# proycon/analiticcl

Hardware: AMD Instinct MI355X
Metric: scored (query,candidate) pairs/sec + queries/sec, 200k-lexicon, len≤16, 1/2/4/8 GPU (higher is better)
Workload: dtype u8

## Files before the change

analiticcl_amd/csrc/engine.hip:

```cpp
#include <hip/hip_runtime.h>

#include <algorithm>
#include <atomic>
#include <functional>
#include <chrono>
#include <cmath>
#include <cstdio>
#include <cstdlib>
#include <cstring>
#include <map>
#include <memory>
#include <mutex>
#include <unordered_map>
#include <numeric>
#include <thread>
#include <type_traits>

#include "engine_internal.h"

namespace anx {

#define HIP_TRY(expr)                                                                          \
  do {                                                                                         \
    hipError_t _e = (expr);                                                                    \
// ... 372 lines not shown
  DeviceLexicon* d = new DeviceLexicon();
  d->device = device;
  { DevPool& pl = pool_of(device); std::lock_guard<std::mutex> g(pl.mu); ++pl.lexicons; }
  d->nplanes = img.nplanes;
  d->nsym = img.nsym;
  d->nclasses = img.nclasses;
  d->nentries = img.nentries;
  d->cstride = img.cstride;
  d->any_variants = img.any_variants ? 1 : 0;
  uint32_t maxlen = 1;
  for (uint32_t m : img.ent_meta) maxlen = std::max(maxlen, m & 0xFFu);
  d->max_len = maxlen;
  int rc = ANX_OK;
  std::vector<EntRec> rec(img.ent_vocab.size());
  for (size_t e = 0; e < rec.size(); ++e) rec[e] = EntRec{img.ent_vocab[e], img.ent_freq[e], img.ent_order[e], img.ent_meta[e]};
  std::vector<uint4> erec(2 * img.ent_vocab.size());
  for (size_t e = 0; e < img.ent_vocab.size(); ++e) {
    memcpy(&erec[2 * e], &img.rows[(size_t)img.ent_rowoff[e] * 16], 16);
    erec[2 * e + 1] = make_uint4(img.ent_meta[e], img.ent_rowoff[e], img.ent_freq[e], 0u);
  }
  std::vector<uint4> eplanes(img.ent_vocab.size());
  for (size_t e = 0; e < img.ent_vocab.size(); ++e) {
    uint32_t pw[3];
    symbol_planes16(&img.rows[(size_t)img.ent_rowoff[e] * 16], img.ent_meta[e] & 0xFFu, pw);
    eplanes[e] = make_uint4(img.ent_meta[e], pw[0], pw[1], pw[2]);
  }
  std::vector<uint4> srec((size_t)img.nentries + 1, make_uint4(0u, 0u, 0u, 0u));
  std::vector<uint2> srec34((size_t)img.nentries + 1, make_uint2(0u, 0u));
  for (uint32_t c = 0; c < img.nclasses; ++c)
    for (uint32_t e = img.cls_off[c]; e < img.cls_off[c + 1]; ++e) {
      srec[e] = make_uint4(img.cls_bits[c], img.cls_bits[(size_t)img.cstride + c], img.cls_len[c], c);
      srec34[e] = make_uint2(img.cls_bits[2 * (size_t)img.cstride + c], img.cls_bits[3 * (size_t)img.cstride + c]);
    }
  srec[img.nentries] = make_uint4(0u, 0u, 255u, 0xFFFFFFFFu);
// ... 922 lines not shown
    if (surv_fill) {
      CompactArgs ca{m.have_freq ? 1 : 0, dl->any_variants};
      hipLaunchKernelGGL(k_compact, dim3(((surv_fill + 255) / 256) * SCAN_REGIONS), dim3(256), 0, st, b->surv, b->sctr,
                         (uint32_t)b->surv_region_cap, ca, b->qcur, dl->ent_rec, dl->ent_var_off, dl->var_target,
                         dl->var_target_freq, dl->var_score, b->c_rows);
    }
  } else if (b->surv_cap == 0 && (rc = ensure_surv(b, b->hint_rows ? b->hint_rows : (size_t)nq * 16 / cap_div() + 1024, err))) return rc;
  const uint32_t row_cap = (uint32_t)std::min<size_t>(b->surv_cap, 0xFFFFFFFFu);
  if (!dl->any_variants)
    hipLaunchKernelGGL(k_compact_grouped, dim3(COMPACT_P * SCAN_REGIONS), dim3(COMPACT_B), 0, st, b->surv, b->sctr,
                       (uint32_t)b->surv_region_cap, m.have_freq ? 1 : 0, b->qcur, dl->ent_rec, b->c_rows, b->soff + nq, row_cap,
                       b->counters + CTR_OVERFLOW);
  HIP_TRY(hipEventRecord(b->ev[3], st));
  if (b->conf_mode == 2 && (rc = conf_launch(m, dl, b, st, true, row_cap, err))) return rc;
  launch_rank(ra, st, nq, b->soff, b->c_rows, b->qmaxfreq, b->qexpand, b->t_key, b->r_rows, b->r_count, dl->any_variants ? 0xFFFFFFFFu : row_cap, b->counters + CTR_OVERFLOW,
              dl->any_variants ? SegRows{nullptr, 0u, nullptr} : SegRows{so.seg, so.seg_cap, dl->ent_rec});
  if (b->conf_mode == 1 && (rc = conf_launch(m, dl, b, st, false, row_cap, err))) return rc;
  exclusive_scan(b->r_count, nq, b->r_off, b->scan_tmp, st, b->counters + CTR_MAXROWS);
  HIP_TRY(hipEventRecord(b->ev[4], st));
  return ANX_OK;
}

int Run::readback() {
  HIP_TRY(hipMemcpyAsync(b->h_read + HR_SCTR, b->sctr, SCAN_REGIONS * RC_STRIDE * sizeof(uint32_t), hipMemcpyDeviceToHost, st));
  HIP_TRY(hipMemcpyAsync(b->h_read + HR_LCTR, b->lctr, 3 * SCAN_REGIONS * RC_STRIDE * sizeof(uint32_t), hipMemcpyDeviceToHost, st));
  HIP_TRY(hipMemcpyAsync(b->h_read + HR_CTR, b->counters, CTR_N * sizeof(uint32_t), hipMemcpyDeviceToHost, st));
  HIP_TRY(hipMemcpyAsync(b->h_read + HR_TOTAL_SURV, b->soff + nq, sizeof(uint32_t), hipMemcpyDeviceToHost, st));
  HIP_TRY(hipMemcpyAsync(b->h_read + HR_TOTAL_RESULTS, b->r_off + nq, sizeof(uint32_t), hipMemcpyDeviceToHost, st));
  b->h_read[HR_CONF] = b->h_read[HR_CONF + 1] = 0;
  if (b->conf_mode && b->cf_ctr) HIP_TRY(hipMemcpyAsync(b->h_read + HR_CONF, b->cf_ctr, 2 * sizeof(uint32_t), hipMemcpyDeviceToHost, st));
  HIP_TRY(hipEventRecord(b->ev_done, st));
// ... 476 lines not shown
```

analiticcl_amd/csrc/host_model.cpp:

```cpp
#include "host_model.h"
#include "adjacency.h"

#include <sched.h>

#include <thread>

#include <algorithm>
#include <cmath>
#include <cstdio>
#include <cstring>
#include <fstream>
#include <numeric>
#include <sstream>

#include "unicode_tables.inc"

namespace anx {

static std::vector<uint32_t> make_primes() {
  std::vector<uint32_t> p;
  for (uint32_t n = 2; p.size() < 168; ++n) {
    bool prime = true;
    for (uint32_t d : p) {
      if (d * d > n) break;
// ... 488 lines not shown

namespace {
struct SwitchDef { const char* name; void (*set)(Switches&, const char*); };
int flag01(const char* v, int dflt) { return !v ? dflt : (v[0] == '0' ? 0 : 1); }
const SwitchDef kSwitches[] = {
    {"ANX_ENCODE", [](Switches& s, const char* v) { s.encode_host = v && strcmp(v, "host") == 0; }},
    {"ANX_SCAN", [](Switches& s, const char* v) { s.scan_sad = v && strcmp(v, "sad") == 0; }},
    {"ANX_SCAN_WALK", [](Switches& s, const char* v) { s.scan_walk_flat = v && strcmp(v, "flat") == 0; }},
    {"ANX_SCAN_TQ", [](Switches& s, const char* v) { const int x = v ? atoi(v) : 0; s.scan_tq = x >= 1 && x <= 64 ? x : 0; }},
    {"ANX_SCAN_ADJ", [](Switches& s, const char* v) { s.scan_adj = flag01(v, 1); }},
    {"ANX_ADJ_BUILD", [](Switches& s, const char* v) { s.adj_build_host = v && strcmp(v, "host") == 0; }},
    {"ANX_ADJ_CLOSURE", [](Switches& s, const char* v) { const int x = v ? atoi(v) : 2; s.adj_closure = x >= 0 && x <= kAdjMaxClosure ? x : kAdjMaxClosure; }},
    {"ANX_SCAN_CHUNK_FUSED", [](Switches& s, const char* v) { const int x = v ? atoi(v) : 0; s.scan_chunk_fused = x >= 32 && x <= 1024 ? x : 0; }},
    {"ANX_ADJ_FAIL", [](Switches& s, const char* v) { s.adj_fail = flag01(v, 0); }},
    {"ANX_SMALL", [](Switches& s, const char* v) { s.small_path = flag01(v, 1); }},
    {"ANX_SURV_SEG", [](Switches& s, const char* v) { const int x = v ? atoi(v) : 32; s.surv_seg = x >= 0 && x <= 256 ? x : 32; }},
    {"ANX_ENC_PRIORITY", [](Switches& s, const char* v) { s.enc_priority = flag01(v, 1); }},
    {"ANX_HINTS", [](Switches& s, const char* v) { s.hints = flag01(v, 1); }},
    {"ANX_ADJ_MB", [](Switches& s, const char* v) { const long x = v ? atol(v) : 0; s.adj_budget_mb = x > 0 ? x : 16384; }},
    {"ANX_SIG_GROUPS", [](Switches& s, const char* v) { const int x = v ? atoi(v) : 0; s.sig_groups = x >= 1 && x <= 8 ? x : 0; }},
    {"ANX_PREFILTER", [](Switches& s, const char* v) { s.prefilter = flag01(v, 1); }},
    {"ANX_SCORE_FAST", [](Switches& s, const char* v) { s.score_fast = flag01(v, 1); }},
    {"ANX_FS_SPLIT", [](Switches& s, const char* v) { s.fs_split = flag01(v, 1); }},
    {"ANX_FS_PLANES", [](Switches& s, const char* v) { s.fs_planes = flag01(v, 1); }},
    {"ANX_FS_B7", [](Switches& s, const char* v) { s.fs_b7 = flag01(v, 1); }},
    {"ANX_SCAN_FUSE", [](Switches& s, const char* v) { s.fuse_prefilter = flag01(v, 1); }},
    {"ANX_CAP_DIV", [](Switches& s, const char* v) { const long x = v ? atol(v) : 0; s.cap_div = x > 1 ? x : 1; }},
    {"ANX_MAX_BATCH", [](Switches& s, const char* v) { const long x = v ? atol(v) : 0; s.max_batch = x > 0 ? x : (4l << 20); }},
    {"ANX_RUN_OVERLAP", [](Switches& s, const char* v) { s.run_overlap = (v && atoi(v) == 0 && v[0] == '0') ? 0 : 1; }},
    {"ANX_SHARD_POLICY", [](Switches& s, const char* v) { s.shard_by_length = (v && strcmp(v, "range") == 0) ? 0 : 1; }},
// ... 184 lines not shown
    std::vector<uint32_t> byval(lex.nclasses);
    std::iota(byval.begin(), byval.end(), 0u);
    std::sort(byval.begin(), byval.end(), [&](uint32_t a, uint32_t b) { return lex.cls_value[a].cmp(lex.cls_value[b]) < 0; });
    lex.ent_order.assign(lex.nentries, 0);
    uint32_t pos = 0;
    for (uint32_t r : byval)
      for (uint32_t e = lex.cls_off[r]; e < lex.cls_off[r + 1]; ++e) lex.ent_order[e] = pos++;
  }
  for (int c = 0; c <= kMaxSymbols; ++c) lex.bucket_begin[c + 1] += lex.bucket_begin[c];
  for (int c = 0; c <= kMaxSymbols; ++c) lex.siglen_begin[c + 1] += lex.siglen_begin[c];
  lex.nsigs = (uint32_t)lex.sig_lo.size();
  const size_t nsig_pad = ((size_t)lex.nsigs + 63) / 64 * 64 + 64;
  lex.sig_lo.resize(nsig_pad, 0xFFFFFFFFu);
  lex.sig_hi.resize(nsig_pad, 0xFFFFFFFFu);
  lex.sig_cbeg.resize(nsig_pad + 1, lex.nclasses);
  build_lm();
  index_generation.fetch_add(1, std::memory_order_release);
  built = true;
  return ANX_OK;
}

bool HostModel::into_ngram(uint64_t vocab_id, std::vector<uint64_t>& out) const {
  out.clear();
  if (vocab_id >= decoder.size()) return false;
  const std::string& text = decoder[vocab_id].text;
  const size_t tokencount = (size_t)std::count(text.begin(), text.end(), ' ') + 1;
  if (tokencount > 5) return false;
  size_t pos = 0;
  for (;;) {
    const size_t e = text.find(' ', pos);
    const std::string tok = text.substr(pos, e == std::string::npos ? std::string::npos : e - pos);
    auto it = encoder.find(tok);
    out.push_back(it == encoder.end() ? 2 : it->second);
    if (e == std::string::npos) break;
// ... 74 lines not shown
```

analiticcl_amd/csrc/host_model.h:

```cpp
#pragma once
#include <cstdint>
#include <atomic>
#include <memory>
#include <mutex>
#include <string>
#include <unordered_map>
#include <vector>

#include "../../include/anx.h"
#include "confusables_core.hpp"
#include "contextrules_flat.hpp"

namespace anx {

constexpr int kMaxSymbols = 255;
constexpr int kMaxAlphabet = 166;
constexpr int kMaxAnagramDistance = 12;
constexpr int kMaxEditDistance = 12;

struct AlphabetMember {
  std::string bytes;
  int nchars;
};

// ... 50 lines not shown
  int search_onepass = 1;
  int scan_chunk_fused = 0;
  int adj_fail = 0;
  int small_path = 1;
  int enc_priority = 1;
  int hints = 1;
  int encode_timing = 0;
  int search_timing = 0;
  int search_parts = 4;
  long search_parts_min = 2l << 20;
  long search_part_bytes = 4l << 20;
  int search_prio = 1;
  int search_early_output = 1;
  int search_first_pct = 50;
  int surv_seg = 32;
  int learn_fold_host = 0;
  int learn_hash_bits = 63;
};
Switches& switches();
bool set_switch(const char* name, const char* value);

struct VariantRef {
  bool variant_of;
  uint64_t id;
  double score;
};

struct VocabEntry {
  std::string text;
  std::vector<uint8_t> norm;
// ... 13 lines not shown
  std::string to_decimal() const;
};

struct LexiconImage {
  int nsym = 0;
  int nplanes = 0;
  uint32_t nclasses = 0, nentries = 0;
  std::vector<uint32_t> cls_planes;
  uint32_t cstride = 0;
  std::vector<uint32_t> cls_bits;
  std::vector<uint8_t> cls_len;
  std::vector<uint32_t> cls_off;
  uint32_t bucket_begin[kMaxSymbols + 2];
  std::vector<uint32_t> ent_vocab;
  std::vector<uint32_t> ent_freq;
  std::vector<uint32_t> ent_meta;
  std::vector<uint32_t> ent_var_off;
  std::vector<uint32_t> var_target;
  std::vector<uint32_t> var_target_freq;
  std::vector<double> var_score;
  bool any_variants = false;
  std::vector<uint32_t> ent_rowoff;
  std::vector<uint32_t> ent_order;
  std::vector<uint8_t> rows;
  std::vector<BigVal> cls_value;
  std::vector<uint8_t> sym_group;
  uint32_t nsigs = 0;
  std::vector<uint32_t> sig_lo, sig_hi;
  std::vector<uint32_t> sig_cbeg;
  uint32_t siglen_begin[kMaxSymbols + 2];
// ... 129 lines not shown
```

analiticcl_amd/csrc/index_cache.cpp:

```cpp
#include <algorithm>
#include <cstdio>
#include <cstring>

#include "host_model.h"

namespace anx {
namespace {

constexpr char kMagic[8] = {'A', 'N', 'X', 'I', 'D', 'X', '0', '3'};

struct Writer {
  FILE* f;
  bool ok = true;
  void raw(const void* p, size_t n) { if (ok && n && fwrite(p, 1, n, f) != n) ok = false; }
  template <typename T> void pod(const T& v) { raw(&v, sizeof v); }
  void str(const std::string& s) { pod<uint64_t>(s.size()); raw(s.data(), s.size()); }
  template <typename T> void vec(const std::vector<T>& v) { pod<uint64_t>(v.size()); raw(v.data(), v.size() * sizeof(T)); }
};
struct Reader {
  FILE* f;
  bool ok = true;
  void raw(void* p, size_t n) { if (ok && n && fread(p, 1, n, f) != n) ok = false; }
  template <typename T> void pod(T& v) { raw(&v, sizeof v); }
  void str(std::string& s) {
// ... 157 lines not shown
    lex = LexiconImage();
    built = false;
    err = path + " is truncated or corrupt";
    return ANX_EIO;
  }
  encoder.clear();
  encoder.reserve(decoder.size() * 2);
  for (size_t id = 0; id < decoder.size(); ++id) encoder.emplace(decoder[id].text, (uint64_t)id);
  class_of_cv.clear();
  class_of_cv.reserve((size_t)x.nclasses * 2);
  std::string cv((size_t)x.nplanes * 4, '\0');
  for (uint32_t c = 0; c < x.nclasses; ++c) {
    for (int p = 0; p < x.nplanes; ++p) memcpy(&cv[(size_t)p * 4], &x.cls_planes[(size_t)p * x.cstride + c], 4);
    class_of_cv.emplace(cv, c);
  }
  build_lm();
  index_generation.fetch_add(1, std::memory_order_release);
  built = true;
  return ANX_OK;
}

int index_read_tag(const std::string& path, std::string* tag, std::string& err) {
  FILE* f = fopen(path.c_str(), "rb");
  if (!f) { err = "cannot open " + path; return ANX_EIO; }
  Reader r{f};
  char magic[8];
  r.raw(magic, sizeof magic);
  uint32_t groups = 0;
  r.pod(groups);
  std::string fp;
// ... 9 lines not shown
```

analiticcl_amd/csrc/kernels_common.hpp:

```cpp
#pragma once

struct Tile {
  uint32_t q0, nq;
  uint32_t s0, s1;
  uint32_t k;
  uint32_t lq;
  uint32_t sig_lo, sig_hi;
  uint32_t kind;
  uint32_t d;
  uint32_t kend;
  uint32_t ball0, balln;
  uint32_t adj;
  uint32_t flags;
};
constexpr uint32_t BALL_MAX = 4096;
constexpr uint32_t SIG_BYTE_MAX = 120;

constexpr int kSymbolPlanesMaxA = 61;
__host__ __device__ inline void symbol_planes16(const uint8_t* row, uint32_t len, uint32_t (&w)[3]) {
  uint32_t p[6] = {0u, 0u, 0u, 0u, 0u, 0u};
  for (uint32_t i = 0; i < 16u && i < len; ++i) {
    const uint32_t v = (uint32_t)row[i] + 1u;
    for (uint32_t b = 0; b < 6u; ++b) p[b] |= ((v >> b) & 1u) << i;
  }
// ... 73 lines not shown
  uint4* sig = nullptr;
  uint32_t* sig_cbeg = nullptr;
  uint32_t* ent_vocab = nullptr;
  uint32_t* ent_freq = nullptr;
  uint32_t* ent_meta = nullptr;
  uint32_t* ent_rowoff = nullptr;
  uint32_t* ent_order = nullptr;
  EntRec* ent_rec = nullptr;
  uint4* e_rec = nullptr;
  uint4* e_planes = nullptr;
  uint32_t* ent_var_off = nullptr;
  uint32_t* var_target = nullptr;
  uint32_t* var_target_freq = nullptr;
  double* var_score = nullptr;
  int any_variants = 0;
  uint4* rows = nullptr;
  DevAlphabet alpha;
  size_t bytes = 0;
  double* quot = nullptr;
  mutable RunHints hints;
  mutable struct DeviceLm* dlm = nullptr;
  mutable struct DeviceConf* dconf = nullptr;
};

enum { CTR_SKIPPED = 2, CTR_MAXROWS = 3 , CTR_OVERFLOW = 4 , CTR_N = 8 };

struct SurvRow {
  double score;
  unsigned long long ord;
  uint32_t vocab, freq;
  uint32_t via, pad;
};
struct SurvRec {
  uint32_t q, e;
  double score;
};
struct SurvSeg {
  double score;
  uint32_t e, pad;
};
struct DevRow {
  uint32_t vocab_id, via;
  double dist_score, freq_score;
};

struct Batch {
  int device = 0;
  size_t nq = 0;
  anx_params params;
  std::vector<uint32_t> order;
  std::vector<int32_t> status;
  size_t n_input = 0;
  std::vector<Tile> tiles;
  uint32_t ntiles = 0;
  uint32_t n_sad_tiles = 0;
// ... 97 lines not shown
```

analiticcl_amd/csrc/kernels_rank.hpp:

```cpp
#pragma once

struct CompactArgs {
  int have_freq, any_variants;
};
__global__ __launch_bounds__(256) void k_compact(const SurvRec* __restrict__ surv, const uint32_t* __restrict__ sctr,
                                                 uint32_t region_cap, CompactArgs a,
                                                 uint32_t* __restrict__ qcur, const EntRec* __restrict__ ent_rec,
                                                 const uint32_t* __restrict__ ent_var_off,
                                                 const uint32_t* __restrict__ var_target,
                                                 const uint32_t* __restrict__ var_target_freq,
                                                 const double* __restrict__ var_score, SurvRow* __restrict__ c_rows) {
  const uint32_t region = blockIdx.x % SCAN_REGIONS, i = (blockIdx.x / SCAN_REGIONS) * 256 + threadIdx.x;
  const bool live = i < sctr[region * RC_STRIDE];
  if (!live) return;
  const SurvRec sr = surv[(size_t)region * region_cap + i];
  const double s = sr.score;
  const uint32_t e = sr.e, q = sr.q;
  const EntRec er = ent_rec[e];
  const uint32_t f = a.have_freq ? er.freq : 1u;
  const unsigned long long ord = (unsigned long long)er.order << 20;
  uint32_t v0 = 0, v1 = 0, self = 1;
  if (a.any_variants) {
    v0 = ent_var_off[e];
    v1 = ent_var_off[e + 1];
// ... 104 lines not shown
  }
}

struct RankArgs {
  double cutoff_threshold;
  uint64_t max_matches;
  float freq_weight;
  int have_freq, any_variants;
};
constexpr int RANK_LCAP = 128;

struct SegRows {
  const SurvSeg* seg;
  uint32_t cap;
  const EntRec* ent_rec;
};
__device__ __forceinline__ SurvRow row_of(const SurvRow* __restrict__ c_rows, const SegRows& sr, int have_freq, uint32_t q, uint32_t seg0, uint32_t i) {
  if (i < sr.cap) {
    const uint4 g = *reinterpret_cast<const uint4*>(sr.seg + (size_t)q * sr.cap + i);
    const EntRec er = sr.ent_rec[g.z];
    return SurvRow{__longlong_as_double((long long)((unsigned long long)g.x | (unsigned long long)g.y << 32)), (unsigned long long)er.order << 20,
                   er.vocab, have_freq ? er.freq : 1u, 0xFFFFFFFFu, 0u};
  }
  return c_rows[seg0 + i - sr.cap];
}
__device__ __forceinline__ unsigned long long rank_key1(double score) {
  const unsigned long long b = (unsigned long long)__double_as_longlong(score + 0.0);
  return (b >> 63) ? ~b : b | (1ull << 63);
}
__device__ __forceinline__ unsigned long long rank_key2(uint32_t freq, unsigned long long ord) {
// ... 343 lines not shown
    if (a.cutoff_threshold >= 1.0) {
      bool have = false;
      double best = 0.0;
      for (uint32_t i = 0; i < len; ++i) {
        const double sc = result_score(rr[i].dist_score, rr[i].freq_score, fw);
        if (have) {
          if (sc <= best / a.cutoff_threshold) { cutoff = i; break; }
        } else { best = sc; have = true; }
      }
    }
    if (cutoff > 0) len = cutoff;
    r_count[q] = len;
  }
}

constexpr int RANK_QPW = 4;
constexpr int RANK_WAVE_BYTES = RANK_LCAP * 22 + 64 * 16;
template <bool SIMPLE>
__global__ __launch_bounds__(256) void k_rank(uint32_t nq, const uint32_t* __restrict__ soff,
                                              const SurvRow* __restrict__ c_rows,
                                              const uint32_t* __restrict__ qmaxfreq,
                                              const uint32_t* __restrict__ qexpand, RankArgs aa,
                                              double* __restrict__ t_key, DevRow* __restrict__ r_rows,
                                              uint32_t* __restrict__ r_count, uint32_t row_cap, const uint32_t* __restrict__ overflow,
                                              SegRows sr) {
  RankArgs a = aa;
  if (SIMPLE) { a.any_variants = 0; a.freq_weight = 0.0f; }
  __shared__ __attribute__((aligned(16))) uint8_t s_raw[4 * RANK_WAVE_BYTES];
  if (soff[nq] > row_cap || *overflow) return;
  const int lane = threadIdx.x & 63, wid = threadIdx.x >> 6;
  uint8_t* wl = s_raw + wid * RANK_WAVE_BYTES;
  const uint32_t qbase = (blockIdx.x * 4 + wid) * RANK_QPW;
  uint32_t my_seg0 = 0, my_n = 0, my_maxf = 0, my_qex = 0;
  if (lane < RANK_QPW && qbase + lane < nq) {
    my_seg0 = soff[qbase + lane];
    my_n = soff[qbase + lane + 1] - my_seg0;
    my_maxf = qmaxfreq[qbase + lane];
    if (a.any_variants) my_qex = qexpand[qbase + lane];
  }
  uint32_t nmax = my_n;
  nmax = max(nmax, (uint32_t)__shfl_xor((int)nmax, 1));
  nmax = max(nmax, (uint32_t)__shfl_xor((int)nmax, 2));
  nmax = (uint32_t)__builtin_amdgcn_readfirstlane((int)nmax);
  {
    const int grp = lane >> 4, gl = lane & 15;
    uint8_t* gb = wl + grp * 608;
    const uint32_t ng = (uint32_t)__shfl((int)my_n, grp);
    rank_query<16, 16>(qbase + grp, qbase + grp < nq && ng <= 16u, gl, grp * 16, 16u, reinterpret_cast<double*>(gb),
                       reinterpret_cast<unsigned long long*>(gb + 128), reinterpret_cast<uint32_t*>(gb + 256),
                       reinterpret_cast<uint16_t*>(gb + 320), reinterpret_cast<double*>(gb + 352), reinterpret_cast<double*>(gb + 480),
                       (uint32_t)__shfl((int)my_seg0, grp), ng, (uint32_t)__shfl((int)my_maxf, grp),
                       (uint32_t)__shfl((int)my_qex, grp), c_rows, sr, a, t_key, r_rows, r_count);
  }
  if (nmax > 16) {
    __builtin_amdgcn_fence(__ATOMIC_SEQ_CST, "workgroup");
    uint32_t mask32 = 0;
    for (int k = 0; k < RANK_QPW; ++k) {
      const uint32_t nk = (uint32_t)__builtin_amdgcn_readlane((int)my_n, k);
      if (qbase + k < nq && nk > 16u && nk <= 32u) mask32 |= 1u << k;
    }
    while (mask32) {
      const int k0 = __ffs((int)mask32) - 1;
      mask32 &= mask32 - 1u;
      const int k1 = mask32 ? __ffs((int)mask32) - 1 : -1;
      if (k1 >= 0) mask32 &= mask32 - 1u;
      const int half = lane >> 5, gl = lane & 31, kk = half ? k1 : k0;
      const bool valid = kk >= 0;
      const int src = valid ? kk : 0;
      uint8_t* gb = wl + half * 1216;
      rank_query<32, 32>(qbase + (uint32_t)src, valid, gl, half * 32, 32u, reinterpret_cast<double*>(gb),
                         reinterpret_cast<unsigned long long*>(gb + 256), reinterpret_cast<uint32_t*>(gb + 512),
                         reinterpret_cast<uint16_t*>(gb + 640), reinterpret_cast<double*>(gb + 704), reinterpret_cast<double*>(gb + 960),
                         (uint32_t)__shfl((int)my_seg0, src), (uint32_t)__shfl((int)my_n, src), (uint32_t)__shfl((int)my_maxf, src),
                         (uint32_t)__shfl((int)my_qex, src), c_rows, sr, a, t_key, r_rows, r_count);
// ... 186 lines not shown
```

analiticcl_amd/csrc/kernels_score.hpp:

```cpp
#pragma once

struct ScoreArgs {
  const double* quot;
  int dbg;
  int store_pairs;
  double w_ld, w_lcs, w_prefix, w_suffix, w_case, w_sum;
  double score_threshold;
  int have_freq, any_variants;
  uint32_t lqp, lcp;
  uint32_t stride;
  uint32_t qw;
};

struct SurvOut {
  SurvRec* list;
  uint32_t* ctr;
  uint32_t region_cap;
  SurvSeg* seg;
  uint32_t seg_cap;
};
__device__ __forceinline__ bool seg_store(const SurvOut& o, bool keep, uint32_t pos, uint32_t q, uint32_t e, double score) {
  if (!keep || pos >= o.seg_cap) return keep;
  const unsigned long long sb = (unsigned long long)__double_as_longlong(score);
  *reinterpret_cast<uint4*>(o.seg + (size_t)q * o.seg_cap + pos) = make_uint4((uint32_t)sb, (uint32_t)(sb >> 32), e, 0u);
  return false;
}
__device__ inline void surv_append(const SurvOut& o, uint32_t region, bool keep, uint32_t q, uint32_t e, double score, uint32_t seg_pos = 0xFFFFFFFFu) {
  keep = seg_store(o, keep, seg_pos, q, e, score);
  const unsigned long long km = __ballot(keep);
  if (!km) return;
  const uint32_t lane = threadIdx.x & 63;
  uint32_t base = 0;
  if (lane == (uint32_t)__ffsll((long long)km) - 1u) base = atomicAdd(&o.ctr[region * RC_STRIDE], (uint32_t)__popcll(km));
  base = (uint32_t)__builtin_amdgcn_readlane((int)base, __ffsll((long long)km) - 1);
  const uint32_t pos = base + (uint32_t)__popcll(km & ((1ull << lane) - 1ull));
  if (keep && pos < o.region_cap) o.list[(size_t)region * o.region_cap + pos] = SurvRec{q, e, score};
}

__device__ inline double score_finish(int lq, uint32_t ld, uint32_t lcs, uint32_t pre, uint32_t suf, uint32_t qm, uint32_t em, uint32_t q, uint32_t e,
                                      const ScoreArgs& a, uint32_t freq, const uint32_t* __restrict__ ent_var_off,
                                      uint32_t* __restrict__ qmaxfreq, uint32_t* __restrict__ qsurv, uint32_t* __restrict__ qexpand,
                                      uint32_t& samecase, bool& keep, const double* quot17 = nullptr, uint32_t* rows_out = nullptr,
                                      uint32_t* seg_pos = nullptr);
// ... 380 lines not shown
  const uint32_t* ent_meta;
  const uint32_t* ent_rowoff;
  const uint4* rows;
  const uint32_t* ent_freq;
  const uint32_t* ent_var_off;
  double* p_score;
  uint32_t* p_meta;
  uint32_t* qmaxfreq;
  uint32_t* qsurv;
  uint32_t* qexpand;
  const uint4* e_planes;
};

template <int NW>
struct PairRegs {
  uint32_t q = 0, e = 0, qm = 0, em = 0, freq = 1;
  int lq = 0, lc = 0, d = 0;
  uint32_t S[NW], T[NW];
};
template <int NW>
__device__ inline void load_pair_qe(uint32_t q, uint32_t e, bool active, const PairArgs& A, const ScoreArgs& a, PairRegs<NW>& r);
template <int NW>
__device__ inline void load_pair(uint32_t p, bool active, const PairArgs& A, const ScoreArgs& a, PairRegs<NW>& r) {
  uint2 rp = make_uint2(0u, 0u);
  if (active) rp = A.raw[p];
  load_pair_qe<NW>(rp.x, rp.y & RAW_ENTRY_MASK, active, A, a, r);
}
template <int NW>
__device__ inline void load_pair_qe(uint32_t q, uint32_t e, bool active, const PairArgs& A, const ScoreArgs& a, PairRegs<NW>& r) {
#pragma unroll
  for (int w = 0; w < NW; ++w) { r.S[w] = 0xFEFEFEFEu; r.T[w] = 0xFFFFFFFFu; }
  if (!active) return;
  r.q = q;
  r.e = e;
  const uint4 Q0 = rec32(A.q_rec, r.q)[0], QM = rec32(A.q_rec, r.q)[1];
  const uint4 C0 = rec32(A.e_rec, r.e)[0], CM = rec32(A.e_rec, r.e)[1];
  r.qm = QM.x;
  r.em = CM.x;
  r.freq = a.have_freq ? CM.z : 1u;
  r.lq = r.qm & 0xFF; r.d = (r.qm >> 16) & 0xFF; r.lc = r.em & 0xFF;
  r.S[0] = Q0.x; r.S[1] = Q0.y; r.S[2] = Q0.z; r.S[3] = Q0.w;
  r.T[0] = C0.x; r.T[1] = C0.y; r.T[2] = C0.z; r.T[3] = C0.w;
  const uint4* qr = A.q_rows + (size_t)r.q * a.qw;
  const uint4* cr = A.rows + CM.y;
#pragma unroll
  for (int w = 1; w < NW / 4; ++w) {
    if (w * 16 < r.lq) { const uint4 Q = qr[w]; r.S[4 * w] = Q.x; r.S[4 * w + 1] = Q.y; r.S[4 * w + 2] = Q.z; r.S[4 * w + 3] = Q.w; }
    if (w * 16 < r.lc) { const uint4 C = cr[w]; r.T[4 * w] = C.x; r.T[4 * w + 1] = C.y; r.T[4 * w + 2] = C.z; r.T[4 * w + 3] = C.w; }
  }
}
template <int D, int NW>
__device__ inline uint32_t dl_of_pair(const PairRegs<NW>& r, bool active) {
  int lqmax = active ? r.lq : 0;
#pragma unroll
// ... 5 lines not shown
}
template <int NW>
__device__ inline void tail_of_pair(uint32_t p, bool has, uint32_t ld, const PairRegs<NW>& r, const PairArgs& A, const ScoreArgs& a,
                                    const SurvOut& so, uint32_t surv_region, uint32_t* __restrict__ lds) {
  uint32_t lcs = 0, pre = 0, suf = 0, samecase = 1, pos = 0xFFFFFFFFu;
  double score = __builtin_nan("");
  bool keep = false;
  if (has && !(ANX_DBG(a.dbg) & 2)) {
    uint32_t* mine = lds + (threadIdx.x & 255) * (2 * NW + 1);
#pragma unroll
    for (int w = 0; w < NW; ++w) { mine[w] = r.S[w]; mine[NW + w] = r.T[w]; }
    score = score_tail(reinterpret_cast<const uint8_t*>(mine), reinterpret_cast<const uint8_t*>(mine + NW), r.lq, r.lc, ld, r.qm,
                       r.em, r.q, r.e, a, A.ent_freq, A.ent_var_off, A.qmaxfreq, A.qsurv, A.qexpand, lcs, pre, suf, samecase, keep,
                       &pos);
  }
  surv_append(so, surv_region, keep, r.q, r.e, score, pos);
  if (has) {
    if (a.store_pairs) {
      A.p_score[p] = score;
      A.p_meta[p] = ld | (samecase << 7) | (lcs << 8) | (pre << 16) | (suf << 24);
    }
  }
}

template <int D, class MT>
__device__ __forceinline__ bool tail16(uint32_t p, bool has, uint32_t ld, const MT& dm, int lq, int lc, uint32_t qm, uint32_t em, uint32_t q, uint32_t e, uint32_t freq,
                                       const PairArgs& A, const ScoreArgs& a, const double* quot17, double& score, bool want_pos, uint32_t& pos) {
  uint32_t lcs = 0, pre = 0, suf = 0, samecase = 1;
  score = __builtin_nan("");
  bool keep = false;
  if (!(ANX_DBG(a.dbg) & 2)) {
// ... 68 lines not shown
  __syncthreads();
  const uint32_t lane = threadIdx.x & 63;
  auto drain = [&]() {
    asm volatile("s_waitcnt lgkmcnt(0)" ::: "memory");
    const uint32_t m = nsv;
    const bool want_pos = so.seg_cap != 0u;
    uint32_t nk = 0;
    for (uint32_t r0 = 0; r0 < m; r0 += 64) {
      const uint32_t i = r0 + lane;
      const bool active = i < m;
      const uint2 ent = active ? *reinterpret_cast<const uint2*>(&s_sv[i]) : make_uint2(0u, 0u);
      const uint32_t p = p0 + (active ? (uint32_t)s_svoff[i] : 0u), ld = (ent.y >> 26) & 3u;
      const uint32_t q = ent.x, e = ent.y & 0x3FFFFFFu;
      double score;
      bool keep;
      uint32_t pos = 0xFFFFFFFFu;
      if (PL) {
        uint4 qp = make_uint4(0u, 0u, 0u, 0u), cp = qp;
        uint32_t freq = 1u;
        if (active) {
          qp = rec32(A.q_rec, q)[1];
          cp = A.e_planes[e];
          if (a.have_freq) freq = A.ent_freq[e];
        }
        const int lq = qp.x & 0xFF, d = (qp.x >> 16) & 0xFF, lc = cp.x & 0xFF;
        const bool has = active && ld <= (uint32_t)d;
        if (a.store_pairs && active && !has) A.p_meta[p] = PAIR_NONE | (1u << 7);
        PlaneMasks<DD> dm;
        dm.build(qp, cp, has ? lq : 0);
        keep = tail16<DD>(p, has, ld, dm, lq, lc, qp.x, cp.x, q, e, freq, A, a, have_quot ? s_quot : nullptr, score, want_pos, pos);
      } else {
        PairRegs<4> r;
        load_pair_qe<4>(q, e, active && !(ANX_DBG(a.dbg) & 64), A, a, r);
        if (ANX_DBG(a.dbg) & 64) { r.lq = 8; r.lc = 8; r.d = 2; }
        const bool has = active && ld <= (uint32_t)r.d;
        if (a.store_pairs && active && !has) A.p_meta[p] = PAIR_NONE | (1u << 7);
        DiagMasks<DD, B7> dm;
        dm.build(r.S, r.T);
        keep = tail16<DD>(p, has, ld, dm, r.lq, r.lc, r.qm, r.em, q, e, r.freq, A, a, have_quot ? s_quot : nullptr, score, want_pos, pos);
      }
      keep = seg_store(so, keep, pos, q, e, score);
      const unsigned long long km = __ballot(keep);
      if (keep) {
        const unsigned long long sb = (unsigned long long)__double_as_longlong(score);
        s_sv[nk + (uint32_t)__popcll(km & ((1ull << lane) - 1ull))] = make_uint4(q, e, (uint32_t)sb, (uint32_t)(sb >> 32));
      }
      nk += (uint32_t)__popcll(km);
    }
    nsv = 0;
    if (nk && !(ANX_DBG(a.dbg) & 32)) {
      asm volatile("s_waitcnt lgkmcnt(0)" ::: "memory");
      uint32_t sbase = 0;
      if (lane == 0) sbase = atomicAdd(&so.ctr[region * RC_STRIDE], nk);
      sbase = (uint32_t)__builtin_amdgcn_readfirstlane((int)sbase);
      uint4* const out = reinterpret_cast<uint4*>(so.list) + (size_t)region * so.region_cap;
      for (uint32_t i = lane; i < nk; i += 64)
// ... 261 lines not shown
        }
        const uint32_t res = R[(lq % NR) * W + (lc - lq + d + 1)];
        if (res <= (uint32_t)d && !(ANX_DBG(a.dbg) & 2)) {
          ld = res;
          score = score_tail(S, T, lq, lc, ld, qm, em, q, e, a, ent_freq, ent_var_off, qmaxfreq, qsurv, qexpand, lcs, pre, suf, samecase, keep,
                             &kpos);
          kq = q; ke = e; kscore = score;
        }
      }
    }
    if (a.store_pairs) {
      A.p_score[p] = score;
      A.p_meta[p] = ld | (samecase << 7) | (lcs << 8) | (pre << 16) | (suf << 24);
    }
  }
  surv_append(so, region, keep, kq, ke, kscore, kpos);
  }
}
__global__ void k_score_pairs(SlotList in, PairArgs A, ScoreArgs a, SurvOut so) {
  extern __shared__ uint32_t lds32[];
  score_pairs_body(in, A, a, so, lds32, blockIdx.x % SCAN_REGIONS, blockIdx.x / SCAN_REGIONS, gridDim.x / SCAN_REGIONS);
}

struct SmallListArgs {
  SlotList lw, l8, lg;
  int do_wide, do_fast8, fastD;
};
template <int D>
__global__ __launch_bounds__(256) void k_small_lists(SmallListArgs L, FilterArgs f, PairArgs A, ScoreArgs a, SurvOut so) {
  extern __shared__ uint32_t lds32[];
  __shared__ uint32_t s_str[D > 0 ? 256 * 17 : 1];
// ... 10 lines not shown
```

analiticcl_amd/csrc/launch_plan.hpp:

```cpp
#pragma once

static inline ScanArgs scan_args_of(const DeviceLexicon* dl) {
  ScanArgs A{};
  A.cls_bits = dl->cls_bits; A.cls_planes = dl->cls_planes; A.scan_rec = dl->scan_rec; A.scan_rec34 = dl->scan_rec34; A.pad_rec = dl->nentries; A.cstride = dl->cstride; A.pad_class = dl->nclasses;
  A.cls_len = dl->cls_len; A.cls_off = dl->cls_off; A.sig = dl->sig; A.sig_e = dl->sig_e; A.sig_cbeg = dl->sig_cbeg; A.sighash = dl->sighash; A.sighash_e = dl->sighash_e; A.hash_mask = dl->hash_mask; A.ball = dl->ball;
  A.adj_hdr = dl->adj_hdr; A.adj_planes = dl->adj_planes; A.adj_ids = dl->adj_ids;
  A.e_rec = dl->e_rec;
  return A;
}
template <typename F>
static inline void with_nplanes(int nplanes, F&& f) {
  switch (nplanes) {
    case 8: f(std::integral_constant<int, 8>{}); break;
    case 16: f(std::integral_constant<int, 16>{}); break;
    case 24: f(std::integral_constant<int, 24>{}); break;
    case 32: f(std::integral_constant<int, 32>{}); break;
    default: f(std::integral_constant<int, 42>{}); break;
  }
}

struct ScorePlan {
  ScoreArgs sa;
  uint32_t threads;
  int fastD;
// ... 77 lines not shown
  else if (pl.fastD == 2) hipLaunchKernelGGL(k_small_lists<2>, grid, dim3(256), dyn, st, L, fa, pa, pl.sa, so);
  else if (pl.fastD == 3) hipLaunchKernelGGL(k_small_lists<3>, grid, dim3(256), dyn, st, L, fa, pa, pl.sa, so);
  else hipLaunchKernelGGL(k_small_lists<0>, grid, dim3(256), dyn, st, L, fa, pa, pl.sa, so);
}

static inline RankArgs rank_args_of(const HostModel& m, const DeviceLexicon* dl, const anx_params& p, double cutoff) {
  RankArgs ra{};
  ra.cutoff_threshold = cutoff;
  ra.max_matches = p.max_matches;
  ra.freq_weight = p.freq_weight;
  ra.have_freq = m.have_freq ? 1 : 0;
  ra.any_variants = dl->any_variants;
  return ra;
}
static inline void launch_rank(const RankArgs& ra, hipStream_t st, uint32_t nq, const uint32_t* soff, const SurvRow* c_rows, const uint32_t* qmaxfreq, const uint32_t* qexpand, double* t_key,
                               DevRow* r_rows, uint32_t* r_count, uint32_t row_cap, const uint32_t* overflow, const SegRows& seg) {
  const dim3 grid((nq + 4 * RANK_QPW - 1) / (4 * RANK_QPW));
  if (!ra.any_variants && ra.freq_weight == 0.0f) hipLaunchKernelGGL(k_rank<true>, grid, dim3(256), 0, st, nq, soff, c_rows, qmaxfreq, qexpand, ra, t_key, r_rows, r_count, row_cap, overflow, seg);
  else hipLaunchKernelGGL(k_rank<false>, grid, dim3(256), 0, st, nq, soff, c_rows, qmaxfreq, qexpand, ra, t_key, r_rows, r_count, row_cap, overflow, seg);
}
```

Before: 54.26 billion.

## Add late ranking path using precomputed tie ranks from segment survivors

Precomputes a per-entry tie rank on the host (by frequency, then lexicon order) and stores it in the entry record and in each survivor segment slot. A new rank_query_late kernel path ranks queries with up to 32 survivors directly from the segment buffer, comparing score keys and tie ranks. This avoids reading the compacted survivor rows and the heavier general tie-breaking, at the cost of extra tie loads in the scoring kernels and a host-side sort at index build. Enabled by default via ANX_RANK_LATE when frequency settings match.

```diff
diff --git a/analiticcl_amd/csrc/engine.hip b/analiticcl_amd/csrc/engine.hip
--- a/analiticcl_amd/csrc/engine.hip
+++ b/analiticcl_amd/csrc/engine.hip
@@ -410,10 +410,12 @@
   int rc = ANX_OK;
   std::vector<EntRec> rec(img.ent_vocab.size());
   for (size_t e = 0; e < rec.size(); ++e) rec[e] = EntRec{img.ent_vocab[e], img.ent_freq[e], img.ent_order[e], img.ent_meta[e]};
+  if (img.ent_tie.size() != img.ent_vocab.size()) { err = "lexicon image without tie ranks"; lexicon_free(d); return nullptr; }
+  d->tie_have_freq = img.have_freq ? 1 : 0;
   std::vector<uint4> erec(2 * img.ent_vocab.size());
   for (size_t e = 0; e < img.ent_vocab.size(); ++e) {
     memcpy(&erec[2 * e], &img.rows[(size_t)img.ent_rowoff[e] * 16], 16);
-    erec[2 * e + 1] = make_uint4(img.ent_meta[e], img.ent_rowoff[e], img.ent_freq[e], 0u);
+    erec[2 * e + 1] = make_uint4(img.ent_meta[e], img.ent_rowoff[e], img.ent_freq[e], img.ent_tie[e]);
   }
   std::vector<uint4> eplanes(img.ent_vocab.size());
   for (size_t e = 0; e < img.ent_vocab.size(); ++e) {
@@ -1366,7 +1368,7 @@
   HIP_TRY(hipEventRecord(b->ev[3], st));
   if (b->conf_mode == 2 && (rc = conf_launch(m, dl, b, st, true, row_cap, err))) return rc;
   launch_rank(ra, st, nq, b->soff, b->c_rows, b->qmaxfreq, b->qexpand, b->t_key, b->r_rows, b->r_count, dl->any_variants ? 0xFFFFFFFFu : row_cap, b->counters + CTR_OVERFLOW,
-              dl->any_variants ? SegRows{nullptr, 0u, nullptr} : SegRows{so.seg, so.seg_cap, dl->ent_rec});
+              dl->any_variants ? SegRows{nullptr, 0u, nullptr} : SegRows{so.seg, so.seg_cap, dl->ent_rec, dl->tie_have_freq == (m.have_freq ? 1 : 0) ? 1u : 0u});
   if (b->conf_mode == 1 && (rc = conf_launch(m, dl, b, st, false, row_cap, err))) return rc;
   exclusive_scan(b->r_count, nq, b->r_off, b->scan_tmp, st, b->counters + CTR_MAXROWS);
   HIP_TRY(hipEventRecord(b->ev[4], st));
diff --git a/analiticcl_amd/csrc/host_model.cpp b/analiticcl_amd/csrc/host_model.cpp
--- a/analiticcl_amd/csrc/host_model.cpp
+++ b/analiticcl_amd/csrc/host_model.cpp
@@ -526,6 +526,7 @@
     {"ANX_SCAN_CHUNK_FUSED", [](Switches& s, const char* v) { const int x = v ? atoi(v) : 0; s.scan_chunk_fused = x >= 32 && x <= 1024 ? x : 0; }},
     {"ANX_ADJ_FAIL", [](Switches& s, const char* v) { s.adj_fail = flag01(v, 0); }},
     {"ANX_SMALL", [](Switches& s, const char* v) { s.small_path = flag01(v, 1); }},
+    {"ANX_RANK_LATE", [](Switches& s, const char* v) { s.rank_late = flag01(v, 1); }},
     {"ANX_SURV_SEG", [](Switches& s, const char* v) { const int x = v ? atoi(v) : 32; s.surv_seg = x >= 0 && x <= 256 ? x : 32; }},
     {"ANX_ENC_PRIORITY", [](Switches& s, const char* v) { s.enc_priority = flag01(v, 1); }},
     {"ANX_HINTS", [](Switches& s, const char* v) { s.hints = flag01(v, 1); }},
@@ -740,10 +741,24 @@
   lex.sig_lo.resize(nsig_pad, 0xFFFFFFFFu);
   lex.sig_hi.resize(nsig_pad, 0xFFFFFFFFu);
   lex.sig_cbeg.resize(nsig_pad + 1, lex.nclasses);
+  lex.have_freq = have_freq;
+  lex.rank_ties();
   build_lm();
   index_generation.fetch_add(1, std::memory_order_release);
   built = true;
   return ANX_OK;
+}
+
+void LexiconImage::rank_ties() {
+  std::vector<uint32_t> by(ent_vocab.size());
+  std::iota(by.begin(), by.end(), 0u);
+  std::sort(by.begin(), by.end(), [&](uint32_t x, uint32_t y) {
+    const uint32_t fx = have_freq ? ent_freq[x] : 1u, fy = have_freq ? ent_freq[y] : 1u;
+    if (fx != fy) return fx > fy;
+    return ent_order[x] < ent_order[y];
+  });
+  ent_tie.resize(by.size());
+  for (size_t i = 0; i < by.size(); ++i) ent_tie[by[i]] = (uint32_t)i;
 }
 
 bool HostModel::into_ngram(uint64_t vocab_id, std::vector<uint64_t>& out) const {
diff --git a/analiticcl_amd/csrc/host_model.h b/analiticcl_amd/csrc/host_model.h
--- a/analiticcl_amd/csrc/host_model.h
+++ b/analiticcl_amd/csrc/host_model.h
@@ -88,6 +88,7 @@
   int search_early_output = 1;
   int search_first_pct = 50;
   int surv_seg = 32;
+  int rank_late = 1;
   int learn_fold_host = 0;
   int learn_hash_bits = 63;
 };
@@ -131,6 +132,9 @@
   uint32_t bucket_begin[kMaxSymbols + 2];
   std::vector<uint32_t> ent_vocab;
   std::vector<uint32_t> ent_freq;
+  bool have_freq = false;
+  std::vector<uint32_t> ent_tie;
+  void rank_ties();
   std::vector<uint32_t> ent_meta;
   std::vector<uint32_t> ent_var_off;
   std::vector<uint32_t> var_target;
diff --git a/analiticcl_amd/csrc/index_cache.cpp b/analiticcl_amd/csrc/index_cache.cpp
--- a/analiticcl_amd/csrc/index_cache.cpp
+++ b/analiticcl_amd/csrc/index_cache.cpp
@@ -195,6 +195,8 @@
     for (int p = 0; p < x.nplanes; ++p) memcpy(&cv[(size_t)p * 4], &x.cls_planes[(size_t)p * x.cstride + c], 4);
     class_of_cv.emplace(cv, c);
   }
+  x.have_freq = have_freq;
+  x.rank_ties();
   build_lm();
   index_generation.fetch_add(1, std::memory_order_release);
   built = true;
diff --git a/analiticcl_amd/csrc/kernels_common.hpp b/analiticcl_amd/csrc/kernels_common.hpp
--- a/analiticcl_amd/csrc/kernels_common.hpp
+++ b/analiticcl_amd/csrc/kernels_common.hpp
@@ -111,6 +111,7 @@
   uint32_t* var_target_freq = nullptr;
   double* var_score = nullptr;
   int any_variants = 0;
+  int tie_have_freq = 0;
   uint4* rows = nullptr;
   DevAlphabet alpha;
   size_t bytes = 0;
@@ -134,8 +135,9 @@
 };
 struct SurvSeg {
   double score;
-  uint32_t e, pad;
-};
+  uint32_t e, tie;
+};
+
 struct DevRow {
   uint32_t vocab_id, via;
   double dist_score, freq_score;
diff --git a/analiticcl_amd/csrc/kernels_rank.hpp b/analiticcl_amd/csrc/kernels_rank.hpp
--- a/analiticcl_amd/csrc/kernels_rank.hpp
+++ b/analiticcl_amd/csrc/kernels_rank.hpp
@@ -142,6 +142,7 @@
   const SurvSeg* seg;
   uint32_t cap;
   const EntRec* ent_rec;
+  uint32_t late = 0;
 };
 __device__ __forceinline__ SurvRow row_of(const SurvRow* __restrict__ c_rows, const SegRows& sr, int have_freq, uint32_t q, uint32_t seg0, uint32_t i) {
   if (i < sr.cap) {
@@ -515,6 +516,75 @@
   }
 }
 
+template <int G>
+__device__ inline void rank_query_late(uint32_t q, bool valid, int gl, int gshift, unsigned long long* __restrict__ s_key, uint32_t* __restrict__ s_tie,
+                                       double* __restrict__ s_sdist, uint32_t seg0, uint32_t n, uint32_t maxf, const SegRows& sr, const RankArgs& a,
+                                       DevRow* __restrict__ r_rows, uint32_t* __restrict__ r_count) {
+  const unsigned long long gmask = G >= 64 ? ~0ull : ((1ull << (G & 63)) - 1ull);
+  if (!valid) n = 0;
+  const bool mine = (uint32_t)gl < n;
+  uint4 g = make_uint4(0u, 0u, 0u, 0u);
+  if (mine) g = *reinterpret_cast<const uint4*>(sr.seg + (size_t)q * sr.cap + (uint32_t)gl);
+  const double score = __longlong_as_double((long long)((unsigned long long)g.x | (unsigned long long)g.y << 32));
+  const bool prune = a.cutoff_threshold >= 1.0;
+  double best = mine ? fmax(-1.0, score) : -1.0;
+#pragma unroll
+  for (int o = G / 2; o; o >>= 1) best = fmax(best, __shfl_xor(best, o));
+  const double thr = best / a.cutoff_threshold;
+  const bool keep = mine && !(prune && score <= thr && score < best);
+  const unsigned long long m = (__ballot(keep) >> gshift) & gmask;
+  const uint32_t pos = (uint32_t)__popcll(m & ((1ull << gl) - 1ull));
+  n = (uint32_t)__popcll(m);
+  const unsigned long long ki = rank_key1(score);
+  const uint32_t ti = g.w;
+  if (keep) { s_key[pos] = ki; s_tie[pos] = ti; }
+  if (valid && n == 0 && gl == 0) r_count[q] = 0;
+  __builtin_amdgcn_fence(__ATOMIC_SEQ_CST, "workgroup");
+  const uint32_t M = a.max_matches == 0 ? n : (uint32_t)min((uint64_t)n, a.max_matches + 1);
+  uint32_t rank = 0xFFFFFFFFu;
+  if (keep) {
+    rank = 0;
+#pragma unroll 2
+    for (uint32_t j = 0; j < n; ++j) {
+      const unsigned long long kj = s_key[j];
+      const uint32_t tj = s_tie[j];
+      rank += (uint32_t)((kj > ki) | ((kj == ki) & (tj < ti)));
+    }
+    if (rank < M) s_sdist[rank] = score;
+  }
+  __builtin_amdgcn_fence(__ATOMIC_SEQ_CST, "workgroup");
+  const bool tail = n != 0;
+  const bool have = tail && (uint32_t)gl < M;
+  const double di = have ? s_sdist[gl] : 0.0;
+  uint32_t len = n;
+  const uint64_t mm = a.max_matches;
+  const bool crop = tail && mm > 0 && (uint64_t)n > mm;
+  double last = 0.0, cropped = 0.0;
+  if (crop) { last = s_sdist[mm - 1]; cropped = s_sdist[mm]; }
+  const unsigned long long lt = (__ballot(have && crop && di < cropped) >> gshift) & gmask;
+  const uint32_t stop_at = lt ? (uint32_t)__ffsll((long long)lt) - 1 : (uint32_t)G;
+  const unsigned long long eq = (__ballot(have && crop && gl >= 1 && (uint32_t)gl <= stop_at && di == cropped) >> gshift) & gmask;
+  if (crop) {
+    if (cropped < last) len = (uint32_t)mm;
+    else {
+      const uint32_t early = eq ? (uint32_t)__ffsll((long long)eq) - 1 : 0;
+      const uint32_t late = lt ? stop_at : 0;
+      if (early > 0) len = early + 1;
+      else if (late > 0) len = late + 1;
+    }
+  }
+  const unsigned long long cut = (__ballot(have && prune && gl >= 1 && (uint32_t)gl < len && di <= thr) >> gshift) & gmask;
+  if (cut) len = (uint32_t)__ffsll((long long)cut) - 1;
+  if (tail && gl == 0) r_count[q] = len;
+  if (keep && rank < M && rank < len) {
+    const uint2 er = *reinterpret_cast<const uint2*>(sr.ent_rec + g.z);
+    const double max_freq = a.have_freq ? (double)maxf : (maxf ? 1.0 : 0.0);
+    const uint32_t fi = a.have_freq ? er.y : 1u;
+    const double ff = (a.have_freq && max_freq > 0.0) ? (double)fi / max_freq : (double)fi;
+    r_rows[seg0 + rank] = DevRow{er.x, 0xFFFFFFFFu, score, ff};
+  }
+}
+
 constexpr int RANK_QPW = 4;
 constexpr int RANK_WAVE_BYTES = RANK_LCAP * 22 + 64 * 16;
 template <bool SIMPLE>
@@ -530,6 +600,7 @@
   __shared__ __attribute__((aligned(16))) uint8_t s_raw[4 * RANK_WAVE_BYTES];
   if (soff[nq] > row_cap || *overflow) return;
   const int lane = threadIdx.x & 63, wid = threadIdx.x >> 6;
+  const bool late = SIMPLE && sr.late && sr.cap;
   uint8_t* wl = s_raw + wid * RANK_WAVE_BYTES;
   const uint32_t qbase = (blockIdx.x * 4 + wid) * RANK_QPW;
   uint32_t my_seg0 = 0, my_n = 0, my_maxf = 0, my_qex = 0;
@@ -547,18 +618,44 @@
     const int grp = lane >> 4, gl = lane & 15;
     uint8_t* gb = wl + grp * 608;
     const uint32_t ng = (uint32_t)__shfl((int)my_n, grp);
-    rank_query<16, 16>(qbase + grp, qbase + grp < nq && ng <= 16u, gl, grp * 16, 16u, reinterpret_cast<double*>(gb),
-                       reinterpret_cast<unsigned long long*>(gb + 128), reinterpret_cast<uint32_t*>(gb + 256),
-                       reinterpret_cast<uint16_t*>(gb + 320), reinterpret_cast<double*>(gb + 352), reinterpret_cast<double*>(gb + 480),
-                       (uint32_t)__shfl((int)my_seg0, grp), ng, (uint32_t)__shfl((int)my_maxf, grp),
-                       (uint32_t)__shfl((int)my_qex, grp), c_rows, sr, a, t_key, r_rows, r_count);
+    bool v16 = qbase + grp < nq && ng <= 16u;
+    const uint32_t gseg0 = (uint32_t)__shfl((int)my_seg0, grp), gmaxf = (uint32_t)__shfl((int)my_maxf, grp);
+    if (late) {
+      const bool vl = v16 && ng <= sr.cap;
+      if (__ballot(vl))
+        rank_query_late<16>(qbase + grp, vl, gl, grp * 16, reinterpret_cast<unsigned long long*>(gb), reinterpret_cast<uint32_t*>(gb + 128),
+                            reinterpret_cast<double*>(gb + 352), gseg0, ng, gmaxf, sr, a, r_rows, r_count);
+      v16 = v16 && !vl;
+    }
+    if (!late || __ballot(v16))
+      rank_query<16, 16>(qbase + grp, v16, gl, grp * 16, 16u, reinterpret_cast<double*>(gb),
+                         reinterpret_cast<unsigned long long*>(gb + 128), reinterpret_cast<uint32_t*>(gb + 256),
+                         reinterpret_cast<uint16_t*>(gb + 320), reinterpret_cast<double*>(gb + 352), reinterpret_cast<double*>(gb + 480),
+                         gseg0, ng, gmaxf, (uint32_t)__shfl((int)my_qex, grp), c_rows, sr, a, t_key, r_rows, r_count);
   }
   if (nmax > 16) {
     __builtin_amdgcn_fence(__ATOMIC_SEQ_CST, "workgroup");
-    uint32_t mask32 = 0;
+    uint32_t mask32 = 0, mask32l = 0;
     for (int k = 0; k < RANK_QPW; ++k) {
       const uint32_t nk = (uint32_t)__builtin_amdgcn_readlane((int)my_n, k);
-      if (qbase + k < nq && nk > 16u && nk <= 32u) mask32 |= 1u << k;
+      if (qbase + k < nq && nk > 16u && nk <= 32u) {
+        if (late && nk <= sr.cap) mask32l |= 1u << k;
+        else mask32 |= 1u << k;
+      }
+    }
+    while (mask32l) {
+      const int k0 = __ffs((int)mask32l) - 1;
+      mask32l &= mask32l - 1u;
+      const int k1 = mask32l ? __ffs((int)mask32l) - 1 : -1;
+      if (k1 >= 0) mask32l &= mask32l - 1u;
+      const int half = lane >> 5, gl = lane & 31, kk = half ? k1 : k0;
+      const bool valid = kk >= 0;
+      const int src = valid ? kk : 0;
+      uint8_t* gb = wl + half * 1216;
+      rank_query_late<32>(qbase + (uint32_t)src, valid, gl, half * 32, reinterpret_cast<unsigned long long*>(gb), reinterpret_cast<uint32_t*>(gb + 256),
+                          reinterpret_cast<double*>(gb + 704), (uint32_t)__shfl((int)my_seg0, src), (uint32_t)__shfl((int)my_n, src),
+                          (uint32_t)__shfl((int)my_maxf, src), sr, a, r_rows, r_count);
+      __builtin_amdgcn_fence(__ATOMIC_SEQ_CST, "workgroup");
     }
     while (mask32) {
       const int k0 = __ffs((int)mask32) - 1;
diff --git a/analiticcl_amd/csrc/kernels_score.hpp b/analiticcl_amd/csrc/kernels_score.hpp
--- a/analiticcl_amd/csrc/kernels_score.hpp
+++ b/analiticcl_amd/csrc/kernels_score.hpp
@@ -19,14 +19,14 @@
   SurvSeg* seg;
   uint32_t seg_cap;
 };
-__device__ __forceinline__ bool seg_store(const SurvOut& o, bool keep, uint32_t pos, uint32_t q, uint32_t e, double score) {
+__device__ __forceinline__ bool seg_store(const SurvOut& o, bool keep, uint32_t pos, uint32_t q, uint32_t e, double score, uint32_t tie) {
   if (!keep || pos >= o.seg_cap) return keep;
   const unsigned long long sb = (unsigned long long)__double_as_longlong(score);
-  *reinterpret_cast<uint4*>(o.seg + (size_t)q * o.seg_cap + pos) = make_uint4((uint32_t)sb, (uint32_t)(sb >> 32), e, 0u);
+  *reinterpret_cast<uint4*>(o.seg + (size_t)q * o.seg_cap + pos) = make_uint4((uint32_t)sb, (uint32_t)(sb >> 32), e, tie);
   return false;
 }
-__device__ inline void surv_append(const SurvOut& o, uint32_t region, bool keep, uint32_t q, uint32_t e, double score, uint32_t seg_pos = 0xFFFFFFFFu) {
-  keep = seg_store(o, keep, seg_pos, q, e, score);
+__device__ inline void surv_append(const SurvOut& o, uint32_t region, bool keep, uint32_t q, uint32_t e, double score, uint32_t seg_pos, uint32_t tie) {
+  keep = seg_store(o, keep, seg_pos, q, e, score, tie);
   const unsigned long long km = __ballot(keep);
   if (!km) return;
   const uint32_t lane = threadIdx.x & 63;
@@ -437,7 +437,7 @@
 
 template <int NW>
 struct PairRegs {
-  uint32_t q = 0, e = 0, qm = 0, em = 0, freq = 1;
+  uint32_t q = 0, e = 0, qm = 0, em = 0, freq = 1, tie = 0;
   int lq = 0, lc = 0, d = 0;
   uint32_t S[NW], T[NW];
 };
@@ -461,6 +461,7 @@
   r.qm = QM.x;
   r.em = CM.x;
   r.freq = a.have_freq ? CM.z : 1u;
+  r.tie = CM.w;
   r.lq = r.qm & 0xFF; r.d = (r.qm >> 16) & 0xFF; r.lc = r.em & 0xFF;
   r.S[0] = Q0.x; r.S[1] = Q0.y; r.S[2] = Q0.z; r.S[3] = Q0.w;
   r.T[0] = C0.x; r.T[1] = C0.y; r.T[2] = C0.z; r.T[3] = C0.w;
@@ -496,7 +497,7 @@
                        r.em, r.q, r.e, a, A.ent_freq, A.ent_var_off, A.qmaxfreq, A.qsurv, A.qexpand, lcs, pre, suf, samecase, keep,
                        &pos);
   }
-  surv_append(so, surv_region, keep, r.q, r.e, score, pos);
+  surv_append(so, surv_region, keep, r.q, r.e, score, pos, r.tie);
   if (has) {
     if (a.store_pairs) {
       A.p_score[p] = score;
@@ -595,7 +596,7 @@
       const uint32_t q = ent.x, e = ent.y & 0x3FFFFFFu;
       double score;
       bool keep;
-      uint32_t pos = 0xFFFFFFFFu;
+      uint32_t pos = 0xFFFFFFFFu, tie = 0u;
       if (PL) {
         uint4 qp = make_uint4(0u, 0u, 0u, 0u), cp = qp;
         uint32_t freq = 1u;
@@ -610,17 +611,19 @@
         PlaneMasks<DD> dm;
         dm.build(qp, cp, has ? lq : 0);
         keep = tail16<DD>(p, has, ld, dm, lq, lc, qp.x, cp.x, q, e, freq, A, a, have_quot ? s_quot : nullptr, score, want_pos, pos);
+        if (keep && pos < so.seg_cap) tie = rec32(A.e_rec, e)[1].w;
       } else {
         PairRegs<4> r;
         load_pair_qe<4>(q, e, active && !(ANX_DBG(a.dbg) & 64), A, a, r);
         if (ANX_DBG(a.dbg) & 64) { r.lq = 8; r.lc = 8; r.d = 2; }
         const bool has = active && ld <= (uint32_t)r.d;
         if (a.store_pairs && active && !has) A.p_meta[p] = PAIR_NONE | (1u << 7);
+        tie = r.tie;
         DiagMasks<DD, B7> dm;
         dm.build(r.S, r.T);
         keep = tail16<DD>(p, has, ld, dm, r.lq, r.lc, r.qm, r.em, q, e, r.freq, A, a, have_quot ? s_quot : nullptr, score, want_pos, pos);
       }
-      keep = seg_store(so, keep, pos, q, e, score);
+      keep = seg_store(so, keep, pos, q, e, score, tie);
       const unsigned long long km = __ballot(keep);
       if (keep) {
         const unsigned long long sb = (unsigned long long)__double_as_longlong(score);
@@ -912,7 +915,9 @@
       A.p_meta[p] = ld | (samecase << 7) | (lcs << 8) | (pre << 16) | (suf << 24);
     }
   }
-  surv_append(so, region, keep, kq, ke, kscore, kpos);
+  uint32_t ktie = 0;
+  if (keep && kpos < so.seg_cap) ktie = rec32(A.e_rec, ke)[1].w;
+  surv_append(so, region, keep, kq, ke, kscore, kpos, ktie);
   }
 }
 __global__ void k_score_pairs(SlotList in, PairArgs A, ScoreArgs a, SurvOut so) {
diff --git a/analiticcl_amd/csrc/launch_plan.hpp b/analiticcl_amd/csrc/launch_plan.hpp
--- a/analiticcl_amd/csrc/launch_plan.hpp
+++ b/analiticcl_amd/csrc/launch_plan.hpp
@@ -115,8 +115,9 @@
   return ra;
 }
 static inline void launch_rank(const RankArgs& ra, hipStream_t st, uint32_t nq, const uint32_t* soff, const SurvRow* c_rows, const uint32_t* qmaxfreq, const uint32_t* qexpand, double* t_key,
-                               DevRow* r_rows, uint32_t* r_count, uint32_t row_cap, const uint32_t* overflow, const SegRows& seg) {
+                               DevRow* r_rows, uint32_t* r_count, uint32_t row_cap, const uint32_t* overflow, SegRows seg) {
   const dim3 grid((nq + 4 * RANK_QPW - 1) / (4 * RANK_QPW));
+  seg.late = (seg.late && seg.cap && switches().rank_late) ? 1u : 0u;
   if (!ra.any_variants && ra.freq_weight == 0.0f) hipLaunchKernelGGL(k_rank<true>, grid, dim3(256), 0, st, nq, soff, c_rows, qmaxfreq, qexpand, ra, t_key, r_rows, r_count, row_cap, overflow, seg);
   else hipLaunchKernelGGL(k_rank<false>, grid, dim3(256), 0, st, nq, soff, c_rows, qmaxfreq, qexpand, ra, t_key, r_rows, r_count, row_cap, overflow, seg);
 }
```

Measured after the change: 54.94 billion (median of 6 runs). +1.2%, better.
